# RQLuo/CDLNet-video

Hardware: AMD Instinct MI355X
Metric: Mpix/s denoised (fwd+bwd) at K=30,M=64,P=7 (higher is better)
Workload: dtype f32 (split-bf16 x3 MFMA, fp32 accumulate, fp32 storage)

## Files before the change

cdlnet-video_amd/csrc/cdl_common.h:

```cpp
#pragma once
#include <atomic>
#include <hip/hip_runtime.h>
#include "../../include/cdlnet_hip.h"

extern __attribute__((visibility("hidden"))) std::atomic<int> cdl_trace_state;
void cdl_trace_launch(const char *file, int line, const char *func);
void cdl_trace_note(const char *fmt, ...) __attribute__((format(printf, 1, 2)));
#define CDL_TRACE_NOTE(...)                                                               \
    do {                                                                                  \
        if (cdl_trace_state.load(std::memory_order_relaxed) != 0) cdl_trace_note(__VA_ARGS__); \
    } while (0)

#define CDL_LAUNCH_CHECK()                                   \
    do {                                                     \
        if (cdl_trace_state.load(std::memory_order_relaxed) != 0)          \
            cdl_trace_launch(__FILE__, __LINE__, __PRETTY_FUNCTION__);     \
        hipError_t e_ = hipGetLastError();                   \
        if (e_ != hipSuccess) return -(int)e_;               \
    } while (0)

__device__ __forceinline__ float cdl_shrink(float u, float t)
{
    float m = fabsf(u) - t;
    m = m > 0.0f ? m : (m != m ? m : 0.0f);
// ... 39 lines not shown
    p.a = u - ca;
    p.sa = cdl_sgn(p.a);
    p.t1 = g1 * lam;
    const float inner = cdl_shrink(p.a, p.t1);
    p.b = (inner - cb) + l1 * p.sa;
    p.t2 = g2 * lam;
    const float mid = cdl_shrink(p.b, p.t2);
    p.m = (mid + cb) - l1 * p.sa;
    p.z = cdl_shrink(p.m, lam);
    return p;
}

__device__ __forceinline__ bool cdl_st_dx(float x, float t) { return x != 0.0f && fabsf(x) - t > 0.0f; }

__device__ __forceinline__ float cdl_prox_csr1_tangent(const cdl_prox1 &p, float lam, float ud, float zpd)
{
    const bool Ga = cdl_st_dx(p.a, p.tg), Gm = cdl_st_dx(p.m, lam);
    return Gm ? (Ga ? ud : zpd) : 0.0f;
}

__device__ __forceinline__ float cdl_prox_csr2_tangent(const cdl_prox2 &p, float lam, float ud, float zpd, float zad)
{
#pragma clang fp contract(off)
    const bool Ga = cdl_st_dx(p.a, p.t1), Gb = cdl_st_dx(p.b, p.t2), Gm = cdl_st_dx(p.m, lam);
    return Gm ? (Gb ? (Ga ? ud - zpd : 0.0f) : zad) : 0.0f;
}

struct cdl_prox_args {
    const float *zp, *za, *lam, *g1, *g2;
    float *u_out;
};

__device__ __forceinline__ float cdl_prox_apply(const cdl_prox_args &px, float u, size_t idx, int row)
{
    if (px.u_out) px.u_out[idx] = u;
    return px.za ? cdl_prox_csr2(u, px.zp[idx], px.za[idx], px.lam[row], px.g1[row], px.g2[row]).z
                 : cdl_prox_csr1(u, px.zp[idx], px.lam[row], px.g1[row]).z;
}

struct cdl_map_args {
    const float *cmap;
    const float *tslope;
};

__device__ __forceinline__ float cdl_map_threshold(float t0, float c, float slope)
{
#pragma clang fp contract(off)
    const float prod = c * slope;
    return t0 + prod;
}

__device__ __forceinline__ float cdl_prox_apply_map(const cdl_prox_args &px, const cdl_map_args &mp, float u, size_t idx,
                                                    int row, int m, int M, float cm)
{
    if (px.u_out) px.u_out[idx] = u;
    const float lam = cdl_map_threshold(px.lam[row], cm, mp.tslope[m]);
    const float g1 = cdl_map_threshold(px.g1[row], cm, mp.tslope[M + m]);
    return px.za ? cdl_prox_csr2(u, px.zp[idx], px.za[idx], lam, g1, cdl_map_threshold(px.g2[row], cm, mp.tslope[2 * M + m])).z
                 : cdl_prox_csr1(u, px.zp[idx], lam, g1).z;
}

__host__ __device__ __forceinline__ int cdl_floordiv(int a, int b)
{
    int q = a / b;
    return (a % b != 0 && ((a < 0) != (b < 0))) ? q - 1 : q;
}

#ifdef CDL_ABLATE
#define CDL_DBG(flags, bit) (((flags) & (bit)) != 0)
#define CDL_DBG_FIELD(decl) decl
#define CDL_DBG_COMMA(x) , x
#else
#define CDL_DBG(flags, bit) (false)
#define CDL_DBG_FIELD(decl)
#define CDL_DBG_COMMA(x)
#endif

struct cdl_options {
    int mfma_analysis, mfma_synthesis, mfma_wgrad, mfma_dense;
    int no_tiled, no_pipelined_synthesis;
    int fused_snake;
    int fused_grid;
    int fused_da;
    int fusedg_bwd_prec;
    int fusedg_strip;
    int scalar_assemble;
    int fused_debug, dense_debug;
    const char *trace_file;
};
const cdl_options &cdl_opts();
bool cdl_exact_fp32();
int cdl_current_device();
int cdl_cu_count();
int cdl_ensure_dynamic_lds(const void *kernel, int bytes);

static inline bool cdl_aligned16(const void *a, const void *b = nullptr, const void *c = nullptr, const void *d = nullptr)
{
    return ((reinterpret_cast<size_t>(a) | reinterpret_cast<size_t>(b) | reinterpret_cast<size_t>(c) |
             reinterpret_cast<size_t>(d)) & 15) == 0;
}

static inline bool cdl_assemble16(int W, const float *out, const float *mask, const float *sub, const float *acc)
{
    return (W & 3) == 0 && cdl_aligned16(out, mask, sub, acc) && !cdl_opts().scalar_assemble;
}

static inline unsigned cdl_persistent_grid(size_t work_items)
{
    size_t cus = (size_t)cdl_cu_count();
    const int cap = cdl_opts().fused_grid;
    if (cap > 0 && (size_t)cap < cus) cus = (size_t)cap;
    return (unsigned)(work_items < cus ? work_items : cus);
}

template <class Batch>
static inline int cdl_pair_batch(Batch *b, const float *const *w1, const float *const *w2, int K, int shift2, int k0)
{
    constexpr int cap = (int)(sizeof(b->wA) / sizeof(b->wA[0]));
    const int nb = K - k0 < cap ? K - k0 : cap;
    *b = Batch{};
    for (int i = 0; i < nb; ++i) {
        const int k = k0 + i;
        b->wA[i] = shift2 == 0 ? w1[(k + 1) % K] : w1[k];
        b->wB[i] = shift2 == 0 ? w2[k] : w2[(k + 1) % K];
    }
    return nb;
}

static inline bool cdl_geom_ok(const cdl_geom *g)
{
    if (!g) return false;
    if (g->N <= 0 || g->C <= 0 || g->M <= 0) return false;
    if (g->D <= 0 || g->H <= 0 || g->W <= 0) return false;
    if (g->Pd <= 0 || g->Ph <= 0 || g->Pw <= 0) return false;
    if (g->sd <= 0 || g->sh <= 0 || g->sw <= 0) return false;
    if (g->pd < 0 || g->ph < 0 || g->pw < 0) return false;
    if (g->D % g->sd || g->H % g->sh || g->W % g->sw) return false;
    return true;
}

static inline bool cdl_bcast_ok(const cdl_bcast *s, int M, size_t per_m)
{
    if (!s || (s->p != 0 && s->p != 1)) return false;
    const long long dm = s->p ? (long long)per_m : 1;
    if (s->m != 0 && s->m != dm) return false;
    const long long dn = s->m ? dm * M : dm;
    return s->n == 0 || s->n == dn;
}

int cdl_tiled_analysis(const cdl_geom *g, const float *x, const float *w, float alpha, const float *zin,
                       const float *gate, const float *tau, float *out, const cdl_prox_args &px, void *stream,
                       const cdl_map_args &mp = cdl_map_args{nullptr, nullptr});
int cdl_tiled_synthesis(const cdl_geom *g, const float *z, const float *gate, const float *w, float alpha,
                        const float *mask, const float *sub, float *out, float *ws, size_t ws_floats,
                        void *stream);
size_t cdl_tiled_synthesis_ws_floats(const cdl_geom *g);
int cdl_mfma_synthesis(const cdl_geom *g, const float *z, const float *gate, const float *w, float alpha,
                       const float *mask, const float *sub, float *out, float *ws, size_t ws_floats, void *stream);
size_t cdl_mfma_synthesis_ws_floats(const cdl_geom *g);
size_t cdl_dense_ws_floats(const cdl_geom *g, int transpose);
size_t cdl_dense_wgrad_ws_floats(const cdl_geom *g);
int cdl_dense_wgrad(const cdl_geom *g, const float *F, const float *gate, const float *x, float alpha, float *dw,
                    float *ws, size_t ws_floats, void *stream);
int cdl_dense_conv(const cdl_geom *g, int transpose, const float *x, const float *in_gate, const float *w,
                   float alpha, const float *add, const float *add_gate, const float *mask, const float *sub,
                   const float *tau, int relu, const float *out_gate, float *out, float *ws, size_t ws_floats,
                   void *stream);
enum { CDL_VGG_PLAIN = 0, CDL_VGG_BIAS = 1, CDL_VGG_POOL = 2, CDL_VGG_DIFF = 3, CDL_VGG_UNPOOL = 4 };
size_t cdl_dense_vgg_workgroups(const cdl_geom *g, int transpose);
int cdl_dense_vgg(const cdl_geom *g, int transpose, int form, const float *x, const float *w, const float *bias,
                  const float *out_gate, float *out, unsigned char *pool_arg, const unsigned char *unpool_arg,
                  const float *fy, float *seed_x, float *seed_y, double *partial, float *ws, size_t ws_floats,
                  void *stream);
int cdl_mfma_analysis(const cdl_geom *g, const float *x, const float *w, float alpha, const float *zin,
                      const float *gate, const float *tau, float *out, const cdl_prox_args &px, float *ws,
                      size_t ws_floats, void *stream, const cdl_map_args &mp = cdl_map_args{nullptr, nullptr});
size_t cdl_mfma_analysis_ws_floats(const cdl_geom *g);
// ... 20 lines not shown
```

cdlnet-video_amd/csrc/cdl_fused2d.hip:

```cpp
#include <atomic>
#include <cstdlib>
#include <type_traits>
#include <mutex>
#include <utility>
#include <vector>

#include "cdl_common.h"
#include "cdl_fused_sweep.h"


namespace {

#include "cdl_wave_dev.h"

typedef __attribute__((ext_vector_type(4))) __bf16 bf16x4;

constexpr int WX = 2;
constexpr int RB = 8;
constexpr int TW = 32 * WX;
constexpr int HALO = 3;
constexpr int RTW = TW + 2 * HALO;
constexpr int RTC = RTW + 2;
constexpr int LDS_W = 32 * 64 * 16;
constexpr int LDS_TAU = 64 * 4;
// ... 1215 lines not shown
    dtau_reduce_block(reinterpret_cast<float (*)[4]>(sm), reinterpret_cast<float (*)[4]>(sm + 256 * 4), block, q.t, M);
}

inline hipStream_t S(void *s) { return reinterpret_cast<hipStream_t>(s); }

inline bool fused_shape_ok(const cdl_geom *g)
{
    if (!cdl_geom_ok(g)) return false;
    if (g->C != 1 || g->D != 1 || g->Pd != 1 || g->sd != 1 || g->sh != 1 || g->sw != 1) return false;
    if (g->Ph != g->Pw || g->Ph > 7 || (g->Ph & 1) == 0 || g->ph != g->Ph / 2 || g->pw != g->Pw / 2) return false;
    if (g->M != 32 && g->M != 64) return false;
    if (blk_image_elems(g->M, g->H, g->W) * 4 >= ((size_t)1 << 31)) return false;
    return true;
}

inline int debug_flags() { return cdl_opts().fused_debug; }

inline int tiles_x(const cdl_geom *g) { return (g->W + TW - 1) / TW; }
template <int WY> inline int tiles_y(const cdl_geom *g) { return (g->H + Shape<WY>::TH - 1) / Shape<WY>::TH; }

struct Flags {
    int prec, rev, lin, lout;
    bool ok;
};
inline Flags parse_flags(int precision)
{
    Flags f;
    f.prec = precision & 15;
    f.rev = (precision >> 4) & 1;
    f.lin = (precision >> 5) & 3;
    f.lout = (precision >> 7) & 3;
    f.ok = (precision >> 9) == 0 && (f.prec == 0 || f.prec == 1 || f.prec == 2) && f.lin <= LAY_BLK16 && f.lout <= LAY_BLK16;
    return f;
}

template <int WY, int MT, int PREC, int MODE, int LIN, int LOUT>
int launch_stage_one(const FusedParams &p, dim3 grid, hipStream_t st)
{
    using G = Shape<WY>;
    if constexpr (MODE == MODE_BWD && G::TH == GW_TH && !(LIN == LAY_BLK && LOUT == LAY_NCHW)) {
        if (p.r2) {
            if (int rc = cdl_ensure_dynamic_lds((const void *)k_stage<MT, PREC, MODE, LIN, LOUT, true, WY>, G::LDS_STAGE + G::LDS_DA)) return rc;
            k_stage<MT, PREC, MODE, LIN, LOUT, true, WY><<<grid, G::NT, G::LDS_STAGE + G::LDS_DA, st>>>(p);
            CDL_LAUNCH_CHECK();
            return 0;
        }
    }
    if (p.r2) return CDL_EUNSUPPORTED;
    if (int rc = cdl_ensure_dynamic_lds((const void *)k_stage<MT, PREC, MODE, LIN, LOUT, false, WY>, G::LDS_STAGE)) return rc;
    k_stage<MT, PREC, MODE, LIN, LOUT, false, WY><<<grid, G::NT, G::LDS_STAGE, st>>>(p);
    CDL_LAUNCH_CHECK();
    return 0;
}

template <int WY, int MT, int PREC, int MODE>
int launch_stage_lay(const FusedParams &p, int lin, int lout, dim3 grid, hipStream_t st)
{
    if (MODE == MODE_FIRST) lin = lout;
#define CDL_LAY_CASE(a, b) if (lin == a && lout == b) return launch_stage_one<WY, MT, PREC, MODE, a, b>(p, grid, st)
    if constexpr (WY == 2 || MODE == MODE_FIRST) CDL_LAY_CASE(LAY_NCHW, LAY_NCHW);
    if constexpr (WY == 2) CDL_LAY_CASE(LAY_BLK, LAY_BLK);
    CDL_LAY_CASE(LAY_BLK16, LAY_BLK16);
    if constexpr (MODE == MODE_FWD) {
        if constexpr (WY == 2) CDL_LAY_CASE(LAY_BLK, LAY_NCHW);
        CDL_LAY_CASE(LAY_BLK16, LAY_NCHW);
    }
    if constexpr (MODE == MODE_BWD) {
        if constexpr (WY == 2) CDL_LAY_CASE(LAY_NCHW, LAY_BLK);
        if constexpr (WY == 2) CDL_LAY_CASE(LAY_BLK, LAY_NCHW);
        CDL_LAY_CASE(LAY_NCHW, LAY_BLK16);
    }
#undef CDL_LAY_CASE
    return CDL_EUNSUPPORTED;
}

template <int WY, int MT, int PREC>
int launch_stage(const FusedParams &p, int mode, int lin, int lout, dim3 grid, hipStream_t st)
{
    if (mode == MODE_FWD) return launch_stage_lay<WY, MT, PREC, MODE_FWD>(p, lin, lout, grid, st);
    if (mode == MODE_FIRST) return launch_stage_lay<WY, MT, PREC, MODE_FIRST>(p, lin, lout, grid, st);
    return launch_stage_lay<WY, MT, PREC, MODE_BWD>(p, lin, lout, grid, st);
}

int stage_grid(const cdl_geom *, const FusedParams &p)
{
    return (int)cdl_persistent_grid((size_t)p.N * p.tilesX * p.tilesY);
}

template <int WY>
int dispatch_stage(const cdl_geom *g, const FusedParams &p, int mode, const Flags &f, hipStream_t st)
{
    dim3 grid((unsigned)stage_grid(g, p));
    if (g->M == 64)
        return f.prec == 0   ? launch_stage<WY, 2, 0>(p, mode, f.lin, f.lout, grid, st)
               : f.prec == 1 ? launch_stage<WY, 2, 1>(p, mode, f.lin, f.lout, grid, st)
                             : launch_stage<WY, 2, 2>(p, mode, f.lin, f.lout, grid, st);
    return f.prec == 0   ? launch_stage<WY, 1, 0>(p, mode, f.lin, f.lout, grid, st)
           : f.prec == 1 ? launch_stage<WY, 1, 1>(p, mode, f.lin, f.lout, grid, st)
                         : launch_stage<WY, 1, 2>(p, mode, f.lin, f.lout, grid, st);
}

int wgrad_grid(const cdl_geom *g)
{
    const size_t tiles = (size_t)g->N * tiles_x(g) * ((g->H + GW_TH - 1) / GW_TH);
    const size_t cus = (size_t)cdl_cu_count();
    return (int)(tiles < cus ? tiles : cus);
}

size_t wgrad_region_floats(const cdl_geom *g) { return (size_t)wgrad_grid(g) * 2 * g->M * 64; }

template <int MT, int PREC, int LAY>
int launch_wgrad_one(const WgradParams &p, int G, hipStream_t st)
{
    const size_t lds = (size_t)WG_THIN_BYTES + (size_t)8 * MT * 2 * IMG_ELEMS * 2;
    if (int rc = cdl_ensure_dynamic_lds((const void *)k_wgrad2d<MT, PREC, LAY>, (int)lds)) return rc;
    k_wgrad2d<MT, PREC, LAY><<<G, 512, lds, st>>>(p);
    CDL_LAUNCH_CHECK();
    return 0;
}

template <int MT, int PREC>
int launch_wgrad(const WgradParams &p, int lay, int G, hipStream_t st)
{
    if (lay == LAY_BLK) return launch_wgrad_one<MT, PREC, LAY_BLK>(p, G, st);
    if (lay == LAY_BLK16) return launch_wgrad_one<MT, PREC, LAY_BLK16>(p, G, st);
    return launch_wgrad_one<MT, PREC, LAY_NCHW>(p, G, st);
}

inline size_t larger(size_t a, size_t b) { return a > b ? a : b; }
template <int WY> inline size_t shape_tiles(const cdl_geom *g) { return (size_t)g->N * tiles_x(g) * tiles_y<WY>(g); }

template <int WY>
FusedParams stage_params(const cdl_geom *g, const Flags &f, const void *frags, float *patches)
{
    FusedParams p = {};
    p.rev = f.rev;
    p.frags = reinterpret_cast<const uint4 *>(frags);
    p.patches = patches; CDL_DBG_FIELD(p.dbg = debug_flags();)
    p.N = g->N; p.H = g->H; p.W = g->W;
    p.tilesX = tiles_x(g); p.tilesY = tiles_y<WY>(g);
    return p;
}

template <int WY>
int iter_fwd(const cdl_geom *g, const float *r, const float *zin, const float *tau, const void *frags, float sgn,
             float *zout, float *patches, unsigned *map_out, int precision, void *stream)
{
    if (!fused_shape_ok(g)) return CDL_EUNSUPPORTED;
    if (!r || !tau || !frags || !zout || !patches || zout == zin) return CDL_EINVAL;
    if (!cdl_aligned16(frags, patches)) return CDL_EUNSUPPORTED;
    const Flags f = parse_flags(precision);
    if (!f.ok) return CDL_EINVAL;
    if ((f.lin && !cdl_aligned16(zin)) || (f.lout && !cdl_aligned16(zout))) return CDL_EUNSUPPORTED;
    FusedParams p = stage_params<WY>(g, f, frags, patches);
    p.r = r; p.zin = zin; p.zout = zout; p.tau = tau; p.map = map_out;
    p.sgn = sgn; p.do_synth = 1;
    return dispatch_stage<WY>(g, p, zin ? MODE_FWD : MODE_FIRST, f, S(stream));
}

int launch_wgrad_reduce(const cdl_geom *g, const WgradReduce &job, hipStream_t st)
{
    k_wgrad_reduce<<<wgrad_reduce_blocks(job, g->M, g->Ph), 1024, 0, st>>>(job, g->M, g->Ph);
    CDL_LAUNCH_CHECK();
    return 0;
}

template <int WY>
int stage_bwd(const cdl_geom *g, const float *thin, const float *base, const unsigned *map, const void *frags,
              float *du_out, float *patches, float *dtau_partial, int do_synth, int precision, const float *r2,
              float alpha, float *dA, float *workspace, void *stream, WgradReduce *defer = nullptr)
{
    if (!fused_shape_ok(g)) return CDL_EUNSUPPORTED;
    if (!thin || !map || !frags || !du_out || !dtau_partial || du_out == base) return CDL_EINVAL;
    if (!cdl_aligned16(frags, patches)) return CDL_EUNSUPPORTED;
    if (do_synth && !patches) return CDL_EINVAL;
    if (r2 && (!dA || !workspace)) return CDL_EINVAL;
    const Flags f = parse_flags(precision);
    if (!f.ok) return CDL_EINVAL;
    if ((f.lin && !cdl_aligned16(base)) || (f.lout && !cdl_aligned16(du_out))) return CDL_EUNSUPPORTED;
    FusedParams p = stage_params<WY>(g, f, frags, patches);
    p.r = thin; p.zin = base; p.map = const_cast<unsigned *>(map); p.zout = du_out; p.dtau = dtau_partial;
    p.sgn = 1.0f; p.do_synth = do_synth ? 1 : 0;
    p.r2 = r2; p.da_partial = workspace;
    int rc = dispatch_stage<WY>(g, p, MODE_BWD, f, S(stream));
    if (rc || !r2) return rc;
    const WgradReduce job = {workspace, stage_grid(g, p), dA, nullptr, alpha, 0.0f, 0};
    if (defer) { *defer = job; return 0; }
    return launch_wgrad_reduce(g, job, S(stream));
}

int wgrad_partials(const cdl_geom *g, const float *X0, const float *T0, float alpha0, float *dw0,
                   const float *X1, const float *T1, float alpha1, float *dw1, float *workspace,
                   int precision, void *stream, WgradReduce *job)
{
    if (!fused_shape_ok(g)) return CDL_EUNSUPPORTED;
    if (!workspace || (!X0 && !X1)) return CDL_EINVAL;
    if ((X0 && (!T0 || !dw0)) || (X1 && (!T1 || !dw1))) return CDL_EINVAL;
    const Flags f = parse_flags(precision);
    if (!f.ok) return CDL_EINVAL;
    if (f.lin && !cdl_aligned16(X0, X1)) return CDL_EUNSUPPORTED;
    WgradParams p = {};
    p.rev = f.rev;
    p.X[0] = X0; p.T[0] = T0; p.X[1] = X1; p.T[1] = T1;
    p.single = (X0 != nullptr) != (X1 != nullptr);
    if (p.single) {
        if (!X0) { X0 = X1; T0 = T1; alpha0 = alpha1; dw0 = dw1; X1 = nullptr; }
        p.X[0] = p.X[1] = X0; p.T[0] = p.T[1] = T0;
    }
    p.partial = workspace;
    p.N = g->N; p.H = g->H; p.W = g->W;
    p.tilesX = tiles_x(g); p.tilesY = (g->H + GW_TH - 1) / GW_TH;
    p.numTiles = p.N * p.tilesX * p.tilesY;
    int G = wgrad_grid(g);
    if (p.single && G > (p.numTiles + 1) / 2) G = (p.numTiles + 1) / 2;
    int rc;
    if (g->M == 64)
        rc = f.prec == 0 ? launch_wgrad<2, 0>(p, f.lin, G, S(stream))
             : f.prec == 1 ? launch_wgrad<2, 1>(p, f.lin, G, S(stream)) : launch_wgrad<2, 2>(p, f.lin, G, S(stream));
    else
        rc = f.prec == 0 ? launch_wgrad<1, 0>(p, f.lin, G, S(stream))
             : f.prec == 1 ? launch_wgrad<1, 1>(p, f.lin, G, S(stream)) : launch_wgrad<1, 2>(p, f.lin, G, S(stream));
    if (rc) return rc;
    *job = WgradReduce{workspace, G, X0 ? dw0 : nullptr, X1 ? dw1 : nullptr, alpha0, alpha1, p.single};
    return 0;
}

template <int WY>
int assemble(const cdl_geom *g, const float *patches, const float *mask, const float *sub, float alpha, float *out,
             float *acc, int acc_add, void *stream)
{
    if (!fused_shape_ok(g)) return CDL_EUNSUPPORTED;
    if (!patches || (!out && !acc)) return CDL_EINVAL;
    const int tx = tiles_x(g), ty = tiles_y<WY>(g);
    if ((size_t)g->N * g->H * g->W >= ((size_t)1 << 20) && cdl_assemble16(g->W, out, mask, sub, acc)) {
        dim3 grid((unsigned)((g->W + 255) / 256), (unsigned)((g->H + 7) / 8), (unsigned)g->N);
        k_assemble_v4<WY><<<grid, 256, 0, S(stream)>>>(patches, mask, sub, alpha, out, g->N, g->H, g->W, tx, ty, acc, acc_add);
        CDL_LAUNCH_CHECK();
    } else if ((size_t)g->N * g->H * g->W >= ((size_t)1 << 20)) {
        dim3 grid((unsigned)((g->W + 255) / 256), (unsigned)((g->H + 3) / 4), (unsigned)g->N);
        k_assemble<4, WY><<<grid, 256, 0, S(stream)>>>(patches, mask, sub, alpha, out, g->N, g->H, g->W, tx, ty, acc, acc_add);
        CDL_LAUNCH_CHECK();
    } else {
        dim3 grid((unsigned)((g->W + 255) / 256), (unsigned)g->H, (unsigned)g->N);
        k_assemble<1, WY><<<grid, 256, 0, S(stream)>>>(patches, mask, sub, alpha, out, g->N, g->H, g->W, tx, ty, acc, acc_add);
        CDL_LAUNCH_CHECK();
    }
    return 0;
}

struct TimingState {
    std::mutex mu;
    std::atomic<bool> on{false};
    struct Pair { hipEvent_t start, stop; int cls, dev; };
    std::vector<Pair> pairs;
    std::vector<std::pair<hipEvent_t, int>> spare;
};
TimingState g_timing;

struct TimingScope {
    hipStream_t st;
    hipEvent_t stop = nullptr;
    TimingScope(int c, hipStream_t s) : st(s)
    {
        if (!g_timing.on.load(std::memory_order_relaxed)) return;
        std::lock_guard<std::mutex> lk(g_timing.mu);
        const int dev = cdl_current_device();
        hipEvent_t ev[2] = {nullptr, nullptr};
        for (int i = 0; i < 2; ++i) {
            for (size_t k = 0; k < g_timing.spare.size() && !ev[i]; ++k)
                if (g_timing.spare[k].second == dev) {
                    ev[i] = g_timing.spare[k].first;
                    g_timing.spare.erase(g_timing.spare.begin() + k);
                }
            if (!ev[i] && hipEventCreate(&ev[i]) != hipSuccess) return;
        }
        (void)hipEventRecord(ev[0], st);
        stop = ev[1];
        g_timing.pairs.push_back({ev[0], ev[1], c, dev});
    }
    ~TimingScope()
    {
        if (stop) (void)hipEventRecord(stop, st);
    }
};

int prep_pairs(const float *const *w1, const float *const *w2, int K, int shift2, void *frags, int M, int P,
               hipStream_t st)
{
    if (!cdl_aligned16(frags)) return CDL_EUNSUPPORTED;
    const int MT = M / 32, threads = 8 * MT * 64;
    const int frag_uint4 = (int)(cdl_fused2d_frag_bytes(M) / 16);
    for (int k0 = 0; k0 < K; k0 += PREP_BATCH) {
        PrepBatch b;
        const int nb = cdl_pair_batch(&b, w1, w2, K, shift2, k0);
        dim3 grid((unsigned)((threads + 255) / 256), (unsigned)nb);
        k_prep_batch<<<grid, 256, 0, st>>>(b, reinterpret_cast<uint4 *>(frags) + (size_t)k0 * frag_uint4, frag_uint4, MT, P);
        CDL_LAUNCH_CHECK();
    }
    return 0;
}

int snake_enabled() { return cdl_opts().fused_snake; }

template <int WY>
int forward_sweep(const cdl_geom *g, int K, const float *yp, const float *mask, const float *tau,
                  const float *const *wA, const float *const *wB, float *const *z, float *const *r,
                  unsigned *const *maps, float *xp, void *frags, float *patches, const Flags &f, void *stream)
{
    const size_t nm = (size_t)g->N * g->M;
    const int L = f.lin;
    int rc = prep_pairs(wA, wB, K, 1, frags, g->M, g->Ph, S(stream));
    if (rc) return rc;
    return cdl_forward_order_sweep(
        K, frags, cdl_fused2d_frag_bytes(g->M), yp, mask, yp, 1.0f, r, xp, snake_enabled(), L, LAY_NCHW,
        [&](int k, const void *fk, const float *thin, bool reversed, int, int lay_out) {
            TimingScope ts(k ? 0 : 3, S(stream));
            return iter_fwd<WY>(g, thin, k ? z[k - 1] : nullptr, tau + k * nm, fk, k ? -1.0f : 1.0f, z[k], patches, maps ? maps[k] : nullptr,
                                f.prec | CDL_LAYOUT_IN(L) | CDL_LAYOUT_OUT(lay_out) | (reversed ? CDL_TILES_REVERSED : 0), stream);
        },
        [&](const float *m, const float *sub, float alpha, float *out) {
            return assemble<WY>(g, patches, m, sub, alpha, out, nullptr, 0, stream);
        });
}

template <int WY>
int backward_sweep(const cdl_geom *g, int K, const float *yp, const float *mask, const float *c,
                   const float *const *wA, const float *const *wB, const float *const *z,
                   const float *const *r, const unsigned *const *maps, const float *g_xp,
                   const float *g_z, float *const *dA,
                   float *const *dB, float *dt, float *du0, float *du1, float *q, void *frags,
                   float *patches, float *dtau_partial, float *wgrad_ws, const Flags &f, float *dyp,
                   float *dtau, void *stream)
{
    const int M = g->M;
    float *du[2] = {du0, du1};
    const int L = f.lin;
    const int sdir = snake_enabled() ? (((K - 1) & 1) ? CDL_TILES_REVERSED : 0) : 0;
    const int wdir = snake_enabled() ? (sdir ^ CDL_TILES_REVERSED) : 0;
    const int sprec = f.prec | sdir, wprec = f.prec | wdir;
    int rc = cdl_fused2d_wgrad(g, z[K - 1], g_xp, 1.0f, dB[0], nullptr, nullptr, 0.0f, nullptr, wgrad_ws,
                               wprec, stream);
    if (rc) return rc;
    const float *thin = g_xp, *base = g_z;
    const size_t fb = cdl_fused2d_frag_bytes(M);
    rc = prep_pairs(wB, wA, K, 0, frags, M, g->Ph, S(stream));
    if (rc) return rc;
    float *ws_a = wgrad_ws, *ws_b = wgrad_ws + wgrad_region_floats(g);
    const int per_img = tiles_x(g) * tiles_y<WY>(g);
    for (int k = K - 1, flip = 0; k >= 0; --k, flip ^= 1) {
        const void *fk = static_cast<const char *>(frags) + (size_t)k * fb;
        float *duk = du[flip];
        const bool ride = Shape<WY>::TH == GW_TH && cdl_opts().fused_da;
        SweepReduce red = {};
        {
            TimingScope ts(1, S(stream));
            rc = stage_bwd<WY>(g, thin, base, maps[k], fk, duk, patches, dtau_partial, k >= 1 || dyp,
                               sprec | CDL_LAYOUT_IN(k == K - 1 ? LAY_NCHW : L) | CDL_LAYOUT_OUT(L),
                               ride ? (k >= 1 ? r[k - 1] : yp) : nullptr, k >= 1 ? -1.0f : 1.0f, dA[k], ws_a, stream, &red.w[0]);
        }
        if (rc) return rc;
        if (ride) red.wblocks[0] = wgrad_reduce_blocks(red.w[0], M, g->Ph);
        red.t = DtauReduce{dtau_partial, c, dt + (size_t)k * 2 * M, dt + (size_t)k * 2 * M + M, g->N, per_img};
        if (dtau) {
            rc = cdl_dtau_per_sample(dtau_partial, g->N, M, per_img, (size_t)per_img * M, 1, M, dtau + (size_t)k * g->N * M, stream);
            if (rc) return rc;
        }
        if (k == 0 && dyp) {
            rc = assemble<WY>(g, patches, nullptr, nullptr, 1.0f, nullptr, dyp, K > 1, stream);
            if (rc) return rc;
        }
        if (k >= 1) {
            rc = assemble<WY>(g, patches, mask, nullptr, -1.0f, q, dyp, k < K - 1, stream);
            if (rc) return rc;
            {
                TimingScope ts(2, S(stream));
                rc = ride ? wgrad_partials(g, z[k - 1], q, 1.0f, dB[k], nullptr, nullptr, 0.0f, nullptr, ws_b,
                                           wprec | CDL_LAYOUT_IN(L), stream, &red.w[1])
                          : wgrad_partials(g, duk, r[k - 1], -1.0f, dA[k], z[k - 1], q, 1.0f, dB[k], ws_b,
                                           wprec | CDL_LAYOUT_IN(L), stream, &red.w[1]);
            }
            thin = q;
        } else if (!ride) {
            rc = wgrad_partials(g, duk, yp, 1.0f, dA[0], nullptr, nullptr, 0.0f, nullptr, ws_b, wprec | CDL_LAYOUT_IN(L), stream,
                                &red.w[1]);
        }
        if (rc) return rc;
        if (k >= 1 || !ride) red.wblocks[1] = wgrad_reduce_blocks(red.w[1], M, g->Ph);
        k_sweep_reduce<<<red.wblocks[0] + red.wblocks[1] + (M + 3) / 4, 1024, 0, S(stream)>>>(red, M, g->Ph);
        CDL_LAUNCH_CHECK();
        base = duk;
    }
    return 0;
}

template <int WY>
int tangent_sweep(const cdl_geom *g, int K, const float *vp, const float *nvp, const float *mask,
                  const float *const *wA, const float *const *wB, const unsigned *const *maps, float *const *zd,
                  float *const *nrd, float *xdp, void *frags, float *patches, float *dtau_partial, const Flags &f,
                  void *stream)
{
    int rc = prep_pairs(wA, wB, K, 1, frags, g->M, g->Ph, S(stream));
    if (rc) return rc;
    return cdl_forward_order_sweep(
        K, frags, cdl_fused2d_frag_bytes(g->M), vp, mask, nvp, -1.0f, nrd, xdp, snake_enabled(), f.lin, LAY_NCHW,
        [&](int k, const void *fk, const float *thin, bool reversed, int lay_in, int lay_out) {
            return stage_bwd<WY>(g, thin, k ? zd[k - 1] : nullptr, maps[k], fk, zd[k], patches, dtau_partial, 1,
                                 f.prec | CDL_LAYOUT_IN(lay_in) | CDL_LAYOUT_OUT(lay_out) | (reversed ? CDL_TILES_REVERSED : 0),
                                 nullptr, 0.0f, nullptr, nullptr, stream);
        },
        [&](const float *m, const float *sub, float alpha, float *out) {
            return assemble<WY>(g, patches, m, sub, alpha, out, nullptr, 0, stream);
        });
}

}

extern "C" {

int cdl_fused2d_supported(const cdl_geom *g) { return fused_shape_ok(g) ? 1 : 0; }

size_t cdl_fused2d_frag_bytes(int M) { return (size_t)2 * (M / 32) * 8 * 64 * 16; }

size_t cdl_fused2d_patch_floats(const cdl_geom *g)
{
    if (!fused_shape_ok(g)) return 0;
    return larger(shape_tiles<2>(g) * Shape<2>::SLAB, shape_tiles<4>(g) * Shape<4>::SLAB);
}

size_t cdl_fused2d_tiles(const cdl_geom *g)
{
    if (!fused_shape_ok(g)) return 0;
    return larger(shape_tiles<2>(g), shape_tiles<4>(g));
}

int cdl_fused2d_prep(const float *wA, const float *wB, void *frags, int M, int P, void *stream)
{
    if (!wA || !wB || !frags || (M != 32 && M != 64) || P < 1 || P > 7 || !(P & 1)) return CDL_EINVAL;
    if (!cdl_aligned16(frags)) return CDL_EUNSUPPORTED;
    const int MT = M / 32, threads = 8 * MT * 64;
    k_prep<<<(threads + 255) / 256, 256, 0, S(stream)>>>(wA, wB, reinterpret_cast<uint4 *>(frags), MT, P);
    CDL_LAUNCH_CHECK();
    return 0;
}

size_t cdl_fused2d_code_bytes(const cdl_geom *g, int layout)
{
    if (!fused_shape_ok(g) || layout < 0 || layout > LAY_BLK16) return 0;
    const size_t per = layout == LAY_NCHW ? lay_image_bytes<LAY_NCHW>(g->M, g->H, g->W)
                     : layout == LAY_BLK ? lay_image_bytes<LAY_BLK>(g->M, g->H, g->W)
                                         : lay_image_bytes<LAY_BLK16>(g->M, g->H, g->W);
    return (size_t)g->N * per;
}

size_t cdl_fused2d_map_words(const cdl_geom *g)
{
    if (!fused_shape_ok(g)) return 0;
    return (size_t)g->N * 4 * g->H * g->W;
}

int cdl_fused2d_support_map(const cdl_geom *g, const float *z, unsigned *map, void *stream)
{
    if (!fused_shape_ok(g)) return CDL_EUNSUPPORTED;
    if (!z || !map) return CDL_EINVAL;
    const size_t total = (size_t)g->N * 2 * g->H * g->W;
    k_support_map<<<(unsigned)((total + 255) / 256), 256, 0, S(stream)>>>(z, map, g->N, g->M, g->H, g->W);
    CDL_LAUNCH_CHECK();
    return 0;
}

int cdl_fused2d_iter_fwd(const cdl_geom *g, const float *r, const float *zin, const float *tau,
                         const void *frags, float sgn, float *zout, float *patches, unsigned *map_out,
                         int precision, void *stream)
{
    return iter_fwd<2>(g, r, zin, tau, frags, sgn, zout, patches, map_out, precision, stream);
}

int cdl_fused2d_stage_bwd(const cdl_geom *g, const float *thin, const float *base, const unsigned *map,
                          const void *frags, float *du_out, float *patches, float *dtau_partial, int do_synth,
                          const float *r2, float alpha, float *dA, float *workspace, int precision, void *stream)
{
    if (!r2 != !dA || !r2 != !workspace) return CDL_EINVAL;
    return stage_bwd<2>(g, thin, base, map, frags, du_out, patches, dtau_partial, do_synth, precision, r2, alpha, dA, workspace,
                        stream);
}

int cdl_fused2d_dtau_reduce(const cdl_geom *g, const float *dtau_partial, const float *c, float *dt0, float *dt1,
                            float *dtau_n, void *stream)
{
    if (!fused_shape_ok(g)) return CDL_EUNSUPPORTED;
    if (!dtau_partial || !dt0 || !dt1) return CDL_EINVAL;
    const int per_img = tiles_x(g) * tiles_y<2>(g);
    const DtauReduce job = {dtau_partial, c, dt0, dt1, g->N, per_img};
    k_dtau_reduce<<<(g->M + 3) / 4, 1024, 0, S(stream)>>>(job, g->M);
    CDL_LAUNCH_CHECK();
    if (!dtau_n) return 0;
    return cdl_dtau_per_sample(dtau_partial, g->N, g->M, per_img, (size_t)per_img * g->M, 1, g->M, dtau_n, stream);
}

size_t cdl_fused2d_wgrad_workspace_floats(const cdl_geom *g)
{
    if (!fused_shape_ok(g)) return 0;
    return 2 * wgrad_region_floats(g);
}

int cdl_fused2d_wgrad(const cdl_geom *g, const float *X0, const float *T0, float alpha0, float *dw0,
                      const float *X1, const float *T1, float alpha1, float *dw1, float *workspace,
                      int precision, void *stream)
{
    WgradReduce job;
    if (int rc = wgrad_partials(g, X0, T0, alpha0, dw0, X1, T1, alpha1, dw1, workspace, precision, stream, &job)) return rc;
    return launch_wgrad_reduce(g, job, S(stream));
}

int cdl_fused2d_assemble(const cdl_geom *g, const float *patches, const float *mask, const float *sub,
                         float alpha, float *out, float *acc, int acc_add, void *stream)
{
    return assemble<2>(g, patches, mask, sub, alpha, out, acc, acc_add, stream);
}

int cdl_fused2d_timing(int enable)
{
    std::lock_guard<std::mutex> lk(g_timing.mu);
    g_timing.on.store(enable != 0, std::memory_order_relaxed);
    if (enable) {
        for (auto &pr : g_timing.pairs) {
            g_timing.spare.push_back({pr.start, pr.dev});
            g_timing.spare.push_back({pr.stop, pr.dev});
        }
        g_timing.pairs.clear();
    }
    return 0;
}

int cdl_fused2d_timing_read(double *ms_sum, int *count)
{
    if (!ms_sum || !count) return CDL_EINVAL;
    std::lock_guard<std::mutex> lk(g_timing.mu);
    for (int c = 0; c < 4; ++c) { ms_sum[c] = 0.0; count[c] = 0; }
    for (auto &pr : g_timing.pairs) {
        float ms = 0.0f;
        hipError_t e = hipEventSynchronize(pr.stop);
        if (e == hipSuccess) e = hipEventElapsedTime(&ms, pr.start, pr.stop);
        if (e != hipSuccess) return -(int)e;
        ms_sum[pr.cls] += ms;
        ++count[pr.cls];
    }
    return 0;
}

int cdl_fused2d_forward(const cdl_geom *g, int K, const float *yp, const float *mask, const float *tau,
                        const float *const *wA, const float *const *wB, float *const *z, float *const *r,
                        unsigned *const *maps, float *xp, void *frags, float *patches, int precision,
                        void *stream)
{
    if (!fused_shape_ok(g)) return CDL_EUNSUPPORTED;
    if (K < 1 || !yp || !tau || !wA || !wB || !z || !xp || !frags || !patches || (K > 1 && !r)) return CDL_EINVAL;
    const Flags f = parse_flags(precision);
    if (!f.ok || f.lout != 0) return CDL_EINVAL;
    if (f.lin == LAY_BLK16)
        return forward_sweep<4>(g, K, yp, mask, tau, wA, wB, z, r, maps, xp, frags, patches, f, stream);
    return forward_sweep<2>(g, K, yp, mask, tau, wA, wB, z, r, maps, xp, frags, patches, f, stream);
}

int cdl_fused2d_tangent(const cdl_geom *g, int K, const float *vp, const float *nvp, const float *mask,
                        const float *const *wA, const float *const *wB, const unsigned *const *maps, float *const *zd,
                        float *const *nrd, float *xdp, void *frags, float *patches, float *dtau_partial, int precision,
                        void *stream)
{
    if (!fused_shape_ok(g)) return CDL_EUNSUPPORTED;
    if (K < 1 || !vp || !nvp || !wA || !wB || !maps || !zd || !xdp || !frags || !patches || !dtau_partial || (K > 1 && !nrd))
        return CDL_EINVAL;
    const Flags f = parse_flags(precision);
    if (!f.ok || f.lout != 0) return CDL_EINVAL;
    if (f.lin == LAY_BLK16) return CDL_EUNSUPPORTED;
    return tangent_sweep<2>(g, K, vp, nvp, mask, wA, wB, maps, zd, nrd, xdp, frags, patches, dtau_partial, f, stream);
}

int cdl_fused2d_backward(const cdl_geom *g, int K, const float *yp, const float *mask, const float *c,
                         const float *const *wA, const float *const *wB, const float *const *z,
                         const float *const *r, const unsigned *const *maps, const float *g_xp,
                         const float *g_z, float *const *dA,
                         float *const *dB, float *dt, float *du0, float *du1, float *q, void *frags,
                         float *patches, float *dtau_partial, float *wgrad_ws, int precision, float *dyp,
                         float *dtau, void *stream)
{
// ... 15 lines not shown
```

cdlnet-video_amd/csrc/cdl_options.hip:

```cpp
#include <atomic>
#include <cstdarg>
#include <cstdio>
#include <cstdlib>
#include <cstring>
#include <fcntl.h>
#include <map>
#include <mutex>
#include <set>
#include <string>
#include <unistd.h>
#include <utility>

#include "cdl_common.h"

namespace {

std::atomic<const cdl_options *> g_opts{nullptr};
std::mutex g_opts_mutex;

std::mutex g_trace_mutex;
bool g_trace_log_on = false;
std::string g_trace_log;
std::set<std::string> g_trace_filed;
std::string g_trace_path;
constexpr size_t TRACE_LOG_MAX = (size_t)16 << 20;
thread_local char t_trace_note[192];

void trace_set_state(const cdl_options *o)
{
    cdl_trace_state.store((g_trace_log_on ? 1 : 0) | ((o && o->trace_file) ? 2 : 0), std::memory_order_relaxed);
}

int env_int(const char *name, int dflt)
{
    const char *e = getenv(name);
    return (e && *e) ? atoi(e) : dflt;
}
int env_flag_off(const char *name)
{
    const char *e = getenv(name);
    return (e && e[0] == '0') ? 0 : 1;
}

const cdl_options *load_options()
{
    cdl_options *o = new cdl_options;
    o->mfma_analysis = env_flag_off("CDL_MFMA_ANALYSIS");
    o->mfma_synthesis = env_flag_off("CDL_MFMA_SYNTHESIS");
    o->mfma_wgrad = env_flag_off("CDL_MFMA_WGRAD");
    o->mfma_dense = env_flag_off("CDL_MFMA_DENSE");
    o->no_tiled = getenv("CDL_NO_TILED") ? 1 : 0;
    o->no_pipelined_synthesis = getenv("CDL_NO_PIPELINED_SYNTHESIS") ? 1 : 0;
    o->fused_snake = env_flag_off("CDL_FUSED_SNAKE");
    o->fused_grid = env_int("CDL_FUSED_GRID", 0);
    o->fused_da = env_flag_off("CDL_FUSED_DA");
    o->scalar_assemble = env_int("CDL_SCALAR_ASSEMBLE", 0) ? 1 : 0;
    o->fusedg_strip = env_int("CDL_FUSEDG_STRIP", 0) ? 1 : 0;
    o->fusedg_bwd_prec = env_int("CDL_FUSEDG_PREC", -1);
    const char *tf = getenv("CDL_TRACE_FILE");
    o->trace_file = (tf && *tf) ? strdup(tf) : nullptr;
#ifdef CDL_ABLATE
    o->fused_debug = env_int("CDL_FUSED_DEBUG", 0);
    o->dense_debug = env_int("CDL_DENSE_DEBUG", 0);
#else
    o->fused_debug = o->dense_debug = 0;
#endif
    {
        std::lock_guard<std::mutex> lk(g_trace_mutex);
        const std::string path = o->trace_file ? o->trace_file : "";
        if (path != g_trace_path) {
            g_trace_filed.clear();
            g_trace_path = path;
        }
        trace_set_state(o);
    }
    return o;
}

thread_local int t_exact_fp32 = 0;

constexpr int MAX_DEV = 64;
std::atomic<int> g_cus[MAX_DEV];
std::mutex g_attr_mutex;
std::map<std::pair<int, const void *>, int> g_attr_bytes;

}

std::atomic<int> cdl_trace_state{-1};

const cdl_options &cdl_opts()
{
    const cdl_options *o = g_opts.load(std::memory_order_acquire);
    if (!o) {
        std::lock_guard<std::mutex> lk(g_opts_mutex);
        o = g_opts.load(std::memory_order_acquire);
        if (!o) {
            o = load_options();
            g_opts.store(o, std::memory_order_release);
        }
    }
    return *o;
}

bool cdl_exact_fp32() { return t_exact_fp32 != 0; }

extern "C" int cdl_set_exact_fp32(int on)
{
    const int prev = t_exact_fp32;
    t_exact_fp32 = on ? 1 : 0;
    return prev;
}

extern "C" int cdl_options_reload(void)
{
    std::lock_guard<std::mutex> lk(g_opts_mutex);
    g_opts.store(load_options(), std::memory_order_release);
    return 0;
}

int cdl_current_device()
{
    int dev = 0;
    return hipGetDevice(&dev) == hipSuccess ? dev : 0;
}

int cdl_cu_count()
{
    const int dev = cdl_current_device();
    if (dev < 0 || dev >= MAX_DEV) return 256;
    int n = g_cus[dev].load(std::memory_order_relaxed);
    if (n <= 0) {
        int v = 0;
        n = (hipDeviceGetAttribute(&v, hipDeviceAttributeMultiprocessorCount, dev) == hipSuccess && v > 0) ? v : 256;
        g_cus[dev].store(n, std::memory_order_relaxed);
    }
    return n;
}

int cdl_ensure_dynamic_lds(const void *kernel, int bytes)
{
    const int dev = cdl_current_device();
    std::lock_guard<std::mutex> lk(g_attr_mutex);
    auto it = g_attr_bytes.find({dev, kernel});
    if (it != g_attr_bytes.end() && it->second >= bytes) return 0;
    hipError_t e = hipFuncSetAttribute(kernel, hipFuncAttributeMaxDynamicSharedMemorySize, bytes);
    if (e != hipSuccess) return -(int)e;
    g_attr_bytes[{dev, kernel}] = bytes;
    return 0;
}

void cdl_trace_note(const char *fmt, ...)
{
    const size_t have = strlen(t_trace_note);
    if (have + 2 >= sizeof(t_trace_note)) return;
    size_t at = have;
    if (have) t_trace_note[at++] = ' ';
    va_list ap;
    va_start(ap, fmt);
    vsnprintf(t_trace_note + at, sizeof(t_trace_note) - at, fmt, ap);
    va_end(ap);
}

void cdl_trace_launch(const char *file, int line, const char *func)
{
    int state = cdl_trace_state.load(std::memory_order_relaxed);
    const cdl_options &o = cdl_opts();
    if (state < 0) state = cdl_trace_state.load(std::memory_order_relaxed);
    if (state > 0) {
        const char *base = strrchr(file, '/');
        std::string rec = std::string(base ? base + 1 : file) + ":" + std::to_string(line) + "\t" + func + "\t" + t_trace_note;
        rec += "\n";
        std::lock_guard<std::mutex> lk(g_trace_mutex);
        if (g_trace_log_on && g_trace_log.size() + rec.size() <= TRACE_LOG_MAX) g_trace_log += rec;
        if (o.trace_file && g_trace_filed.insert(rec).second) {
            const int fd = open(o.trace_file, O_WRONLY | O_APPEND | O_CREAT | O_CLOEXEC, 0644);
            if (fd >= 0) {
                (void)!write(fd, rec.data(), rec.size());
                close(fd);
            }
        }
    }
    t_trace_note[0] = 0;
}

extern "C" int cdl_trace(int on)
{
    const cdl_options &o = cdl_opts();
    std::lock_guard<std::mutex> lk(g_trace_mutex);
    const int prev = g_trace_log_on ? 1 : 0;
    g_trace_log_on = on != 0;
    if (on) g_trace_log.clear();
    trace_set_state(&o);
    return prev;
}

extern "C" size_t cdl_trace_read(char *buf, size_t cap)
{
    std::lock_guard<std::mutex> lk(g_trace_mutex);
    if (buf && cap) {
        const size_t n = g_trace_log.size() < cap - 1 ? g_trace_log.size() : cap - 1;
        memcpy(buf, g_trace_log.data(), n);
        buf[n] = 0;
    }
    return g_trace_log.size();
}
```

Measured before the change: 119.8.

## Overlap weight-gradient kernels with backward stage on a side stream

Moves the per-layer weight-gradient partials and sweep reduction onto a separate non-blocking stream, forked and joined with events. The CU budget is split between the backward stage grid and the wgrad grid (by default three quarters and one quarter), and q, workspace and dtau buffers are double-buffered by iteration parity so consecutive layers can run concurrently. This aims to hide the serial wgrad time behind the main backward stage, but it shrinks each kernel's persistent grid, enlarges the workspace, and adds event synchronisation overhead. It is disabled under graph capture and for small tile counts.

Result: no change. 120.9, median of 6 (+0.9%).

```diff
diff --git a/cdlnet-video_amd/csrc/cdl_common.h b/cdlnet-video_amd/csrc/cdl_common.h
--- a/cdlnet-video_amd/csrc/cdl_common.h
+++ b/cdlnet-video_amd/csrc/cdl_common.h
@@ -145,6 +145,8 @@
     int fused_snake;
     int fused_grid;
     int fused_da;
+    int fused_wgrad_grid;
+    int fused_overlap, fused_overlap_s, fused_overlap_w;
     int fusedg_bwd_prec;
     int fusedg_strip;
     int scalar_assemble;
@@ -156,6 +158,9 @@
 int cdl_current_device();
 int cdl_cu_count();
 int cdl_ensure_dynamic_lds(const void *kernel, int bytes);
+hipStream_t cdl_side_stream();
+bool cdl_events_get(hipEvent_t *ev, int n);
+void cdl_events_put(const hipEvent_t *ev, int n);
 
 static inline bool cdl_aligned16(const void *a, const void *b = nullptr, const void *c = nullptr, const void *d = nullptr)
 {
diff --git a/cdlnet-video_amd/csrc/cdl_fused2d.hip b/cdlnet-video_amd/csrc/cdl_fused2d.hip
--- a/cdlnet-video_amd/csrc/cdl_fused2d.hip
+++ b/cdlnet-video_amd/csrc/cdl_fused2d.hip
@@ -1321,15 +1321,16 @@
     return launch_stage_lay<WY, MT, PREC, MODE_BWD>(p, lin, lout, grid, st);
 }
 
-int stage_grid(const cdl_geom *, const FusedParams &p)
-{
-    return (int)cdl_persistent_grid((size_t)p.N * p.tilesX * p.tilesY);
+int stage_grid(const cdl_geom *, const FusedParams &p, int cap)
+{
+    const int G = (int)cdl_persistent_grid((size_t)p.N * p.tilesX * p.tilesY);
+    return cap > 0 && cap < G ? cap : G;
 }
 
 template <int WY>
-int dispatch_stage(const cdl_geom *g, const FusedParams &p, int mode, const Flags &f, hipStream_t st)
-{
-    dim3 grid((unsigned)stage_grid(g, p));
+int dispatch_stage(const cdl_geom *g, const FusedParams &p, int mode, const Flags &f, hipStream_t st, int grid_cap = 0)
+{
+    dim3 grid((unsigned)stage_grid(g, p, grid_cap));
     if (g->M == 64)
         return f.prec == 0   ? launch_stage<WY, 2, 0>(p, mode, f.lin, f.lout, grid, st)
                : f.prec == 1 ? launch_stage<WY, 2, 1>(p, mode, f.lin, f.lout, grid, st)
@@ -1339,14 +1340,15 @@
                          : launch_stage<WY, 1, 2>(p, mode, f.lin, f.lout, grid, st);
 }
 
-int wgrad_grid(const cdl_geom *g)
+int wgrad_grid(const cdl_geom *g, int cap)
 {
     const size_t tiles = (size_t)g->N * tiles_x(g) * ((g->H + GW_TH - 1) / GW_TH);
-    const size_t cus = (size_t)cdl_cu_count();
+    size_t cus = (size_t)cdl_cu_count();
+    if (cap > 0 && (size_t)cap < cus) cus = (size_t)cap;
     return (int)(tiles < cus ? tiles : cus);
 }
 
-size_t wgrad_region_floats(const cdl_geom *g) { return (size_t)wgrad_grid(g) * 2 * g->M * 64; }
+size_t wgrad_region_floats(const cdl_geom *g) { return (size_t)wgrad_grid(g, -1) * 2 * g->M * 64; }
 
 template <int MT, int PREC, int LAY>
 int launch_wgrad_one(const WgradParams &p, int G, hipStream_t st)
@@ -1407,7 +1409,7 @@
 template <int WY>
 int stage_bwd(const cdl_geom *g, const float *thin, const float *base, const unsigned *map, const void *frags,
               float *du_out, float *patches, float *dtau_partial, int do_synth, int precision, const float *r2,
-              float alpha, float *dA, float *workspace, void *stream, WgradReduce *defer = nullptr)
+              float alpha, float *dA, float *workspace, void *stream, WgradReduce *defer = nullptr, int grid_cap = 0)
 {
     if (!fused_shape_ok(g)) return CDL_EUNSUPPORTED;
     if (!thin || !map || !frags || !du_out || !dtau_partial || du_out == base) return CDL_EINVAL;
@@ -1421,16 +1423,16 @@
     p.r = thin; p.zin = base; p.map = const_cast<unsigned *>(map); p.zout = du_out; p.dtau = dtau_partial;
     p.sgn = 1.0f; p.do_synth = do_synth ? 1 : 0;
     p.r2 = r2; p.da_partial = workspace;
-    int rc = dispatch_stage<WY>(g, p, MODE_BWD, f, S(stream));
+    int rc = dispatch_stage<WY>(g, p, MODE_BWD, f, S(stream), grid_cap);
     if (rc || !r2) return rc;
-    const WgradReduce job = {workspace, stage_grid(g, p), dA, nullptr, alpha, 0.0f, 0};
+    const WgradReduce job = {workspace, stage_grid(g, p, grid_cap), dA, nullptr, alpha, 0.0f, 0};
     if (defer) { *defer = job; return 0; }
     return launch_wgrad_reduce(g, job, S(stream));
 }
 
 int wgrad_partials(const cdl_geom *g, const float *X0, const float *T0, float alpha0, float *dw0,
                    const float *X1, const float *T1, float alpha1, float *dw1, float *workspace,
-                   int precision, void *stream, WgradReduce *job)
+                   int precision, void *stream, WgradReduce *job, int grid_cap = 0)
 {
     if (!fused_shape_ok(g)) return CDL_EUNSUPPORTED;
     if (!workspace || (!X0 && !X1)) return CDL_EINVAL;
@@ -1450,7 +1452,7 @@
     p.N = g->N; p.H = g->H; p.W = g->W;
     p.tilesX = tiles_x(g); p.tilesY = (g->H + GW_TH - 1) / GW_TH;
     p.numTiles = p.N * p.tilesX * p.tilesY;
-    int G = wgrad_grid(g);
+    int G = wgrad_grid(g, grid_cap > 0 ? grid_cap : cdl_opts().fused_wgrad_grid);
     if (p.single && G > (p.numTiles + 1) / 2) G = (p.numTiles + 1) / 2;
     int rc;
     if (g->M == 64)
@@ -1562,6 +1564,67 @@
         });
 }
 
+constexpr int OVERLAP_MIN_TILES_PER_CU = 4;
+constexpr int OVERLAP_WGRAD_CU_DIV = 4;
+
+inline size_t round4(size_t n) { return (n + 3) & ~(size_t)3; }
+inline size_t overlap_q_floats(const cdl_geom *g) { return round4((size_t)g->N * g->H * g->W); }
+
+struct Overlap {
+    bool on = false, joined = true;
+    int gs = 0, gw = 0;
+    hipStream_t main = nullptr, side = nullptr;
+    hipEvent_t ev_q[2], ev_done[2];
+    int begin(const cdl_geom *g, int K, bool ride, size_t tiles, hipStream_t st)
+    {
+        const cdl_options &o = cdl_opts();
+        if (!ride || o.fused_overlap == 0) return 0;
+        hipStreamCaptureStatus cap = hipStreamCaptureStatusNone;
+        if (hipStreamIsCapturing(st, &cap) != hipSuccess || cap != hipStreamCaptureStatusNone) return 0;
+        const int cus = cdl_cu_count();
+        if (o.fused_overlap == 1) {
+            gs = o.fused_overlap_s;
+            gw = o.fused_overlap_w;
+        } else {
+            if (K < 2 || tiles < (size_t)OVERLAP_MIN_TILES_PER_CU * cus) return 0;
+            gw = cus / OVERLAP_WGRAD_CU_DIV;
+            gs = cus - gw;
+        }
+        main = st;
+        side = cdl_side_stream();
+        if (!side) return -(int)hipErrorOutOfMemory;
+        hipEvent_t ev[4];
+        if (!cdl_events_get(ev, 4)) return -(int)hipErrorOutOfMemory;
+        ev_q[0] = ev[0]; ev_q[1] = ev[1]; ev_done[0] = ev[2]; ev_done[1] = ev[3];
+        on = true;
+        return 0;
+    }
+    static int rc_of(hipError_t e) { return e == hipSuccess ? 0 : -(int)e; }
+    int fork(int par)
+    {
+        if (int rc = rc_of(hipEventRecord(ev_q[par], main))) return rc;
+        joined = false;
+        return rc_of(hipStreamWaitEvent(side, ev_q[par], 0));
+    }
+    int done(int par) { return rc_of(hipEventRecord(ev_done[par], side)); }
+    int wait_done(int par) { return rc_of(hipStreamWaitEvent(main, ev_done[par], 0)); }
+    int join(int par)
+    {
+        joined = true;
+        return wait_done(par);
+    }
+    ~Overlap()
+    {
+        if (!on) return;
+        if (!joined) {
+            (void)hipEventRecord(ev_done[0], side);
+            (void)hipStreamWaitEvent(main, ev_done[0], 0);
+        }
+        const hipEvent_t ev[4] = {ev_q[0], ev_q[1], ev_done[0], ev_done[1]};
+        cdl_events_put(ev, 4);
+    }
+};
+
 template <int WY>
 int backward_sweep(const cdl_geom *g, int K, const float *yp, const float *mask, const float *c,
                    const float *const *wA, const float *const *wB, const float *const *z,
@@ -1577,31 +1640,47 @@
     const int sdir = snake_enabled() ? (((K - 1) & 1) ? CDL_TILES_REVERSED : 0) : 0;
     const int wdir = snake_enabled() ? (sdir ^ CDL_TILES_REVERSED) : 0;
     const int sprec = f.prec | sdir, wprec = f.prec | wdir;
-    int rc = cdl_fused2d_wgrad(g, z[K - 1], g_xp, 1.0f, dB[0], nullptr, nullptr, 0.0f, nullptr, wgrad_ws,
-                               wprec, stream);
+    const bool ride = Shape<WY>::TH == GW_TH && cdl_opts().fused_da;
+    const size_t region = wgrad_region_floats(g);
+    float *ws_a[2] = {wgrad_ws, wgrad_ws + 2 * region}, *ws_b = wgrad_ws + region;
+    float *qs[2] = {q, wgrad_ws + 3 * region};
+    float *dtps[2] = {dtau_partial, qs[1] + overlap_q_floats(g)};
+    Overlap ov;
+    int rc = ov.begin(g, K, ride, shape_tiles<WY>(g), S(stream));
+    if (rc) return rc;
+    void *wstream = ov.on ? (void *)ov.side : stream;
+    if (ov.on && (rc = ov.fork(0))) return rc;
+    {
+        WgradReduce job0;
+        rc = wgrad_partials(g, z[K - 1], g_xp, 1.0f, dB[0], nullptr, nullptr, 0.0f, nullptr, ov.on ? ws_b : wgrad_ws, wprec,
+                            wstream, &job0, ov.gw);
+        if (!rc) rc = launch_wgrad_reduce(g, job0, S(wstream));
+    }
     if (rc) return rc;
     const float *thin = g_xp, *base = g_z;
     const size_t fb = cdl_fused2d_frag_bytes(M);
     rc = prep_pairs(wB, wA, K, 0, frags, M, g->Ph, S(stream));
     if (rc) return rc;
-    float *ws_a = wgrad_ws, *ws_b = wgrad_ws + wgrad_region_floats(g);
     const int per_img = tiles_x(g) * tiles_y<WY>(g);
     for (int k = K - 1, flip = 0; k >= 0; --k, flip ^= 1) {
         const void *fk = static_cast<const char *>(frags) + (size_t)k * fb;
         float *duk = du[flip];
-        const bool ride = Shape<WY>::TH == GW_TH && cdl_opts().fused_da;
+        const int par = ov.on ? flip : 0;
+        float *qk = qs[par], *dtp = dtps[par];
+        if (ov.on && k <= K - 3 && (rc = ov.wait_done(par))) return rc;
         SweepReduce red = {};
         {
             TimingScope ts(1, S(stream));
-            rc = stage_bwd<WY>(g, thin, base, maps[k], fk, duk, patches, dtau_partial, k >= 1 || dyp,
+            rc = stage_bwd<WY>(g, thin, base, maps[k], fk, duk, patches, dtp, k >= 1 || dyp,
                                sprec | CDL_LAYOUT_IN(k == K - 1 ? LAY_NCHW : L) | CDL_LAYOUT_OUT(L),
-                               ride ? (k >= 1 ? r[k - 1] : yp) : nullptr, k >= 1 ? -1.0f : 1.0f, dA[k], ws_a, stream, &red.w[0]);
+                               ride ? (k >= 1 ? r[k - 1] : yp) : nullptr, k >= 1 ? -1.0f : 1.0f, dA[k], ws_a[par], stream, &red.w[0],
+                               ov.gs);
         }
         if (rc) return rc;
         if (ride) red.wblocks[0] = wgrad_reduce_blocks(red.w[0], M, g->Ph);
-        red.t = DtauReduce{dtau_partial, c, dt + (size_t)k * 2 * M, dt + (size_t)k * 2 * M + M, g->N, per_img};
+        red.t = DtauReduce{dtp, c, dt + (size_t)k * 2 * M, dt + (size_t)k * 2 * M + M, g->N, per_img};
         if (dtau) {
-            rc = cdl_dtau_per_sample(dtau_partial, g->N, M, per_img, (size_t)per_img * M, 1, M, dtau + (size_t)k * g->N * M, stream);
+            rc = cdl_dtau_per_sample(dtp, g->N, M, per_img, (size_t)per_img * M, 1, M, dtau + (size_t)k * g->N * M, stream);
             if (rc) return rc;
         }
         if (k == 0 && dyp) {
@@ -1609,24 +1688,29 @@
             if (rc) return rc;
         }
         if (k >= 1) {
-            rc = assemble<WY>(g, patches, mask, nullptr, -1.0f, q, dyp, k < K - 1, stream);
+            rc = assemble<WY>(g, patches, mask, nullptr, -1.0f, qk, dyp, k < K - 1, stream);
             if (rc) return rc;
+            if (ov.on && (rc = ov.fork(par))) return rc;
             {
-                TimingScope ts(2, S(stream));
-                rc = ride ? wgrad_partials(g, z[k - 1], q, 1.0f, dB[k], nullptr, nullptr, 0.0f, nullptr, ws_b,
-                                           wprec | CDL_LAYOUT_IN(L), stream, &red.w[1])
-                          : wgrad_partials(g, duk, r[k - 1], -1.0f, dA[k], z[k - 1], q, 1.0f, dB[k], ws_b,
+                TimingScope ts(2, S(wstream));
+                rc = ride ? wgrad_partials(g, z[k - 1], qk, 1.0f, dB[k], nullptr, nullptr, 0.0f, nullptr, ws_b,
+                                           wprec | CDL_LAYOUT_IN(L), wstream, &red.w[1], ov.gw)
+                          : wgrad_partials(g, duk, r[k - 1], -1.0f, dA[k], z[k - 1], qk, 1.0f, dB[k], ws_b,
                                            wprec | CDL_LAYOUT_IN(L), stream, &red.w[1]);
             }
-            thin = q;
+            thin = qk;
+        } else if (ov.on) {
+            rc = ov.fork(par);
         } else if (!ride) {
             rc = wgrad_partials(g, duk, yp, 1.0f, dA[0], nullptr, nullptr, 0.0f, nullptr, ws_b, wprec | CDL_LAYOUT_IN(L), stream,
                                 &red.w[1]);
         }
         if (rc) return rc;
         if (k >= 1 || !ride) red.wblocks[1] = wgrad_reduce_blocks(red.w[1], M, g->Ph);
-        k_sweep_reduce<<<red.wblocks[0] + red.wblocks[1] + (M + 3) / 4, 1024, 0, S(stream)>>>(red, M, g->Ph);
+        k_sweep_reduce<<<red.wblocks[0] + red.wblocks[1] + (M + 3) / 4, 1024, 0, S(wstream)>>>(red, M, g->Ph);
         CDL_LAUNCH_CHECK();
+        if (ov.on && (rc = ov.done(par))) return rc;
+        if (ov.on && k == 0 && (rc = ov.join(par))) return rc;
         base = duk;
     }
     return 0;
@@ -1739,7 +1823,7 @@
 size_t cdl_fused2d_wgrad_workspace_floats(const cdl_geom *g)
 {
     if (!fused_shape_ok(g)) return 0;
-    return 2 * wgrad_region_floats(g);
+    return 3 * wgrad_region_floats(g) + overlap_q_floats(g) + round4(shape_tiles<2>(g) * g->M);
 }
 
 int cdl_fused2d_wgrad(const cdl_geom *g, const float *X0, const float *T0, float alpha0, float *dw0,
diff --git a/cdlnet-video_amd/csrc/cdl_options.hip b/cdlnet-video_amd/csrc/cdl_options.hip
--- a/cdlnet-video_amd/csrc/cdl_options.hip
+++ b/cdlnet-video_amd/csrc/cdl_options.hip
@@ -10,6 +10,7 @@
 #include <string>
 #include <unistd.h>
 #include <utility>
+#include <vector>
 
 #include "cdl_common.h"
 
@@ -54,6 +55,19 @@
     o->fused_snake = env_flag_off("CDL_FUSED_SNAKE");
     o->fused_grid = env_int("CDL_FUSED_GRID", 0);
     o->fused_da = env_flag_off("CDL_FUSED_DA");
+    o->fused_wgrad_grid = env_int("CDL_FUSED_WGRAD_GRID", 0);
+    o->fused_overlap = -1;
+    o->fused_overlap_s = o->fused_overlap_w = 0;
+    if (const char *ov = getenv("CDL_FUSED_OVERLAP"); ov && *ov) {
+        int gs = 0, gw = 0;
+        if (sscanf(ov, "%d:%d", &gs, &gw) == 2 && gs > 0 && gw > 0) {
+            o->fused_overlap = 1;
+            o->fused_overlap_s = gs;
+            o->fused_overlap_w = gw;
+        } else {
+            o->fused_overlap = 0;
+        }
+    }
     o->scalar_assemble = env_int("CDL_SCALAR_ASSEMBLE", 0) ? 1 : 0;
     o->fusedg_strip = env_int("CDL_FUSEDG_STRIP", 0) ? 1 : 0;
     o->fusedg_bwd_prec = env_int("CDL_FUSEDG_PREC", -1);
@@ -84,6 +98,10 @@
 std::mutex g_attr_mutex;
 std::map<std::pair<int, const void *>, int> g_attr_bytes;
 
+std::mutex g_side_mutex;
+hipStream_t g_side_stream[MAX_DEV];
+std::vector<hipEvent_t> g_side_events[MAX_DEV];
+
 }
 
 std::atomic<int> cdl_trace_state{-1};
@@ -147,6 +165,44 @@
     if (e != hipSuccess) return -(int)e;
     g_attr_bytes[{dev, kernel}] = bytes;
     return 0;
+}
+
+hipStream_t cdl_side_stream()
+{
+    const int dev = cdl_current_device();
+    if (dev < 0 || dev >= MAX_DEV) return nullptr;
+    std::lock_guard<std::mutex> lk(g_side_mutex);
+    if (!g_side_stream[dev] && hipStreamCreateWithFlags(&g_side_stream[dev], hipStreamNonBlocking) != hipSuccess)
+        g_side_stream[dev] = nullptr;
+    return g_side_stream[dev];
+}
+
+bool cdl_events_get(hipEvent_t *ev, int n)
+{
+    const int dev = cdl_current_device();
+    if (dev < 0 || dev >= MAX_DEV) return false;
+    std::lock_guard<std::mutex> lk(g_side_mutex);
+    std::vector<hipEvent_t> &pool = g_side_events[dev];
+    int have = 0;
+    for (; have < n; ++have) {
+        if (!pool.empty()) {
+            ev[have] = pool.back();
+            pool.pop_back();
+        } else if (hipEventCreateWithFlags(&ev[have], hipEventDisableTiming) != hipSuccess) {
+            break;
+        }
+    }
+    if (have == n) return true;
+    pool.insert(pool.end(), ev, ev + have);
+    return false;
+}
+
+void cdl_events_put(const hipEvent_t *ev, int n)
+{
+    const int dev = cdl_current_device();
+    if (dev < 0 || dev >= MAX_DEV) return;
+    std::lock_guard<std::mutex> lk(g_side_mutex);
+    g_side_events[dev].insert(g_side_events[dev].end(), ev, ev + n);
 }
 
 void cdl_trace_note(const char *fmt, ...)
```
